# baker-laboratory/NA-MPNN

Measured on AMD Instinct MI355X. Metric: residues/sec (enc+dec fwd), N~1000 K=48 h=128; seq-recovery vs CPU ref, higher is better.
Workload: dtype f32; 1 GPU; cfg2: B=1 x N=1000 residues per rank, K=48, H=128, 3 enc + 3 dec layers, per-edge GEMMs fp32, seeded random-init weights, independent complexes per rank; precision=fp32, global_batch=1, seq_len=1000, parallelism=replicas x1

## Files before the change

na_mpnn_amd/csrc/namp_kernels.h:

```cpp
#pragma once
#include "namp_device.h"
#ifndef NAMP_MAX_LAYERS
#define NAMP_MAX_LAYERS 8
#endif

static __global__ void pack_image_kernel(const float* __restrict__ W, int ld, int col0, int OUT, int IN,
                                  float* __restrict__ img) {
  const int total = OUT * IN;
  for (int e = blockIdx.x * blockDim.x + threadIdx.x; e < total; e += gridDim.x * blockDim.x) {
    const int r = e & 3, lane = (e >> 2) & 63, t = e >> 8;
    const int ntn = OUT >> 4;
    const int tn = t % ntn, tk = t / ntn;
    const int n = 16 * tn + (lane & 15), k = 16 * tk + 4 * (lane >> 4) + r;
    img[e] = W[(size_t)n * ld + col0 + k];
  }
}

static __global__ void pack_image_bf16_kernel(const float* __restrict__ W, int ld, int col0, __bf16* __restrict__ img) {
  const int e = blockIdx.x * blockDim.x + threadIdx.x;
  if (e >= 128 * 128) return;
  const int j = e & 7, lane = (e >> 3) & 63, tn = (e >> 9) & 7, s = e >> 12;
  const int n = 16 * tn + (lane & 15), k = 32 * s + 16 * (j >> 2) + 4 * (lane >> 4) + (j & 3);
  img[e] = (__bf16)W[(size_t)n * ld + col0 + k];
}
// ... 357 lines not shown
        a0 = __builtin_elementwise_fma(w2, (f2){xv[q].x, xv[q].y}, a0);
        a1 = __builtin_elementwise_fma(w2, (f2){xv[q].z, xv[q].w}, a1);
      }
      __builtin_amdgcn_sched_barrier(0);
    }
    acc[0] = a0.x; acc[1] = a0.y; acc[2] = a1.x; acc[3] = a1.y;
    return;
  }
  f2 a2[R / 2];
#pragma unroll
  for (int q = 0; q < R / 2; ++q) a2[q] = (f2){acc[2 * q], acc[2 * q + 1]};
#pragma unroll
  for (int tk = 0; tk < 8; ++tk) {
#pragma unroll
    for (int r = 0; r < 4; ++r) {
      const float* xp = xT + (16 * tk + 4 * g + r) * R;
      const f2 w2 = (f2){wf[tk][r], wf[tk][r]};
#pragma unroll
      for (int q = 0; q < R; q += 4) {
        const f4 xv = *(const f4*)(xp + q);
        a2[q / 2] = __builtin_elementwise_fma(w2, (f2){xv.x, xv.y}, a2[q / 2]);
        a2[q / 2 + 1] = __builtin_elementwise_fma(w2, (f2){xv.z, xv.w}, a2[q / 2 + 1]);
      }
    }
    __builtin_amdgcn_sched_barrier(0);
  }
#pragma unroll
  for (int q = 0; q < R / 2; ++q) { acc[2 * q] = a2[q].x; acc[2 * q + 1] = a2[q].y; }
}

#define ROWS_TAIL_LDS_FLOATS(R) ((128 + 512 + 4 * 128 + 128) * (R) + 64 + 128 * (R))

struct ConsecutiveRows {
  int row0, nrows, G;
  __device__ __forceinline__ int operator()(int n) const { return (n < nrows && row0 + n < G) ? row0 + n : -1; }
};

template <bool SC1>
__device__ __forceinline__ void st_out(float* p, const float v) {
  if (SC1) __hip_atomic_store(p, v, __ATOMIC_RELAXED, __HIP_MEMORY_SCOPE_AGENT);
  else *p = v;
}

template <bool PF, class FragFn, class BodyFn>
__device__ __forceinline__ void tail_units(const int u0, const int total, const int step, const int lane, FragFn frag, BodyFn body,
                                           const int rot = 0) {
  if constexpr (!PF) {
#pragma unroll 1
    for (int u_ = u0; u_ < total; u_ += step) {
      const int u = (u_ + rot) & (total - 1);
      f4 wf[8];
#pragma unroll
      for (int tk = 0; tk < 8; ++tk) wf[tk] = frag(u, tk)[lane];
      body(u, wf);
    }
  } else {
    f4 wa[8], wb[8];
    int u = u0;
    if (u < total) {
#pragma unroll
      for (int tk = 0; tk < 8; ++tk) wa[tk] = frag(u, tk)[lane];
    }
#pragma unroll 1
    while (u < total) {
      int un = u + step;
      if (un < total) {
#pragma unroll
        for (int tk = 0; tk < 8; ++tk) wb[tk] = frag(un, tk)[lane];
      }
      body(u, wa);
      u = un;
      if (u >= total) break;
      un = u + step;
      if (un < total) {
#pragma unroll
        for (int tk = 0; tk < 8; ++tk) wa[tk] = frag(un, tk)[lane];
      }
      body(u, wb);
      u = un;
    }
  }
}

__device__ __forceinline__ int tail4_off(const int k, const int j) { return (((k >> 4) * 4 + ((k >> 2) & 3)) * 4 + j) * 4 + (k & 3); }

template <int NB>
__device__ __forceinline__ void tail4_x(f4 (&xr)[NB][8], const float* xB, const int lane) {
  const float* p = xB + ((lane >> 4) * 4 + (lane & 3)) * 4;
#pragma unroll
  for (int nb = 0; nb < NB; ++nb)
#pragma unroll
    for (int S = 0; S < 8; ++S) xr[nb][S] = *(const f4*)(p + nb * 512 + S * 64);
}

template <int NB>
__device__ __forceinline__ void tail4_unit(f4 (&o)[NB], const f4 (&wf)[8], const f4 (&xr)[NB][8]) {
  f4 c0[NB], c1[NB];
#ifdef NAMP_ABL_T4_NOMFMA
#pragma unroll
  for (int nb = 0; nb < NB; ++nb) {
    o[nb] = (f4){0.f, 0.f, 0.f, 0.f};
#pragma unroll
    for (int S = 0; S < 8; ++S) o[nb] += wf[S] * xr[nb][S];
  }
  return;
#endif
#pragma unroll
  for (int nb = 0; nb < NB; ++nb) { c0[nb] = (f4){0.f, 0.f, 0.f, 0.f}; c1[nb] = (f4){0.f, 0.f, 0.f, 0.f}; }
#pragma unroll
  for (int S = 0; S < 8; ++S) {
#pragma unroll
    for (int nb = 0; nb < NB; ++nb) {
      c0[nb] = __builtin_amdgcn_mfma_f32_4x4x1f32(wf[S].x, xr[nb][S].x, c0[nb], 0, 0, 0);
      c1[nb] = __builtin_amdgcn_mfma_f32_4x4x1f32(wf[S].y, xr[nb][S].y, c1[nb], 0, 0, 0);
    }
#pragma unroll
    for (int nb = 0; nb < NB; ++nb) {
      c0[nb] = __builtin_amdgcn_mfma_f32_4x4x1f32(wf[S].z, xr[nb][S].z, c0[nb], 0, 0, 0);
      c1[nb] = __builtin_amdgcn_mfma_f32_4x4x1f32(wf[S].w, xr[nb][S].w, c1[nb], 0, 0, 0);
    }
  }
#pragma unroll
  for (int nb = 0; nb < NB; ++nb) {
    f4 v = c0[nb] + c1[nb];
#pragma unroll
    for (int c = 0; c < 4; ++c) { v[c] += __shfl_xor(v[c], 16); v[c] += __shfl_xor(v[c], 32); }
    o[nb] = v;
  }
}

#define TAIL4_AHEAD 3
template <class FragFn>
__device__ __forceinline__ void tail4_request1(f4 (&wf)[8], const int u, const int lane, FragFn frag) {
#ifdef NAMP_ABL_T4_NOLOAD
#pragma unroll
  for (int tk = 0; tk < 8; ++tk) wf[tk] = (f4){1.f * u, 2.f * lane, 3.f, 4.f * tk};
  return;
#endif
#pragma unroll
  for (int tk = 0; tk < 8; ++tk) wf[tk] = frag(u, tk)[lane];
}
template <class FragFn>
__device__ __forceinline__ void tail4_request(f4 (&wf)[TAIL4_AHEAD][8], const int u0, const int total, const int step, const int lane, FragFn frag) {
#pragma unroll
  for (int t = 0; t < TAIL4_AHEAD; ++t) {
    const int u = u0 + t * step;
    tail4_request1(wf[t], u < total ? u : u0, lane, frag);
  }
}
template <class FragFn, class BodyFn, class NextFn>
__device__ __forceinline__ void tail4_phase(f4 (&wf)[TAIL4_AHEAD][8], const int u0, const int total, const int step, const int lane, FragFn frag,
                                            BodyFn body, NextFn next) {
#pragma unroll
  for (int t = 0; t < TAIL4_AHEAD; ++t) {
    const int u = u0 + t * step;
    if (u < total) body(u, wf[t]);
    next(t);
  }
  tail_units<false>(u0 + TAIL4_AHEAD * step, total, step, lane, frag, body);
}

template <int R, typename RowFn, bool SC1, bool M3, bool PF, bool AH>
__device__ __forceinline__ void node_tail_mfma4(const NodeTail& a, f4 (&x)[8], const float wsum_m, const RowFn orow, float* lds,
                                                const int tid, const int wave, const int nwaves, const int lane) {
  static_assert(R == 4 || R == 8, "node_tail_mfma4: 4 or 8 rows");
  constexpr int NB = R / 4;
  constexpr bool AHEAD = AH && !PF && R == 4;
  float* xB = lds;
  float* hB = xB + 128 * R;
  float* oP = hB + 512 * R;
  float* yT = oP + 4 * 128 * R;
  float* red = yT + 128 * R;
  float* yB = red + 64;
  const int m = lane & 15, g = lane >> 4;
  const int cb = (lane >> 2) & 3, j = lane & 3;
  const bool st_lane = lane < 16;
  const auto win_frag = [&](const int u, const int tk) { return (const f4*)a.Win_img + (tk * 32 + u) * 64; };
  const auto wout_frag = [&](const int u, const int tk) { return (const f4*)a.Wout_img + ((8 * (u >> 3) + tk) * 8 + (u & 7)) * 64; };

  NAMP_STAMP_BEGIN();
  f4 wa[AHEAD ? TAIL4_AHEAD : 1][8];
  float bin_a[TAIL4_AHEAD] = {0.f, 0.f, 0.f};
  if constexpr (AHEAD) {
    tail4_request(wa, wave, 32, nwaves, lane, win_frag);
#pragma unroll
    for (int t = 0; t < TAIL4_AHEAD; ++t) {
      const int u = wave + t * nwaves;
      bin_a[t] = a.b_in[16 * (u < 32 ? u : wave) + 4 * cb + g];
    }
  }
  if (M3 && a.m3_img) {
    if (wave == 0 && m < R) {
#pragma unroll
      for (int t = 0; t < 8; ++t) *(f4*)(xB + (m >> 2) * 512 + t * 64 + g * 16 + (m & 3) * 4) = x[t];
      if (g == 0) red[m] = wsum_m;
    }
    __syncthreads();
    {
      f4 xr[NB][8];
      tail4_x<NB>(xr, xB, lane);
      tail_units<PF>(wave, 8, nwaves, lane,
                     [&](const int u, const int tk) { return (const f4*)a.m3_img + (tk * 8 + u) * 64; },
                     [&](const int u, const f4 (&wf)[8]) {
                       f4 o[NB];
                       tail4_unit<NB>(o, wf, xr);
                       if (st_lane) {
                         const f4 b = *(const f4*)(a.m3_b + 16 * u + 4 * cb);
#pragma unroll
                         for (int nb = 0; nb < NB; ++nb) *(f4*)(oP + (4 * nb + j) * NAMP_H + 16 * u + 4 * cb) = o[nb] + b * red[4 * nb + j];
                       }
                     });
    }
    __syncthreads();
    const int mr = m < R ? m : 0;
    int hr = orow(mr);
    if (hr < 0) hr = orow(0) < 0 ? 0 : orow(0);
    const float* hsrc = a.hV + (long)hr * NAMP_H + 4 * g;
#pragma unroll
    for (int t = 0; t < 8; ++t) x[t] = *(const f4*)(hsrc + 16 * t) + *(const f4*)(oP + mr * NAMP_H + 16 * t + 4 * g);
  }

  NAMP_STAMP(7);
  layernorm_row_T(x, a.ln1_g, a.ln1_b, g);
  if (wave == 0 && m < R) {
#pragma unroll
    for (int t = 0; t < 8; ++t) *(f4*)(xB + (m >> 2) * 512 + t * 64 + g * 16 + (m & 3) * 4) = x[t];
  }
  __syncthreads();
  NAMP_STAMP(8);
  {
    f4 xr[NB][8];
    tail4_x<NB>(xr, xB, lane);
    const auto body = [&](const int u, const f4 (&wf)[8]) {
      f4 o[NB];
      tail4_unit<NB>(o, wf, xr);
      const int t_ = AHEAD ? (u - wave) / nwaves : 0;
      const float b = (AHEAD && t_ < TAIL4_AHEAD) ? (t_ == 0 ? bin_a[0] : t_ == 1 ? bin_a[1] : bin_a[2]) : a.b_in[16 * u + 4 * cb + g];
#pragma unroll
      for (int nb = 0; nb < NB; ++nb) {
        const float v = g == 0 ? o[nb].x : g == 1 ? o[nb].y : g == 2 ? o[nb].z : o[nb].w;
        hB[((u >> 3) * NB + nb) * 512 + (u & 7) * 64 + cb * 16 + j * 4 + g] = gelu_erf(v + b);
      }
    };
    if constexpr (AHEAD)
      tail4_phase(wa, wave, 32, nwaves, lane, win_frag, body, [&](const int t) {
        const int u = wave + t * nwaves;
        tail4_request1(wa[t], u < 32 ? u : wave, lane, wout_frag);
      });
    else tail_units<PF>(wave, 32, nwaves, lane, win_frag, body);
  }
  __syncthreads();
  NAMP_STAMP(9);
  {
    const auto body = [&](const int u, const f4 (&wf)[8]) {
      const int tn = u & 7, q = u >> 3;
      f4 xr[NB][8];
      tail4_x<NB>(xr, hB + q * NB * 512, lane);
      f4 o[NB];
      tail4_unit<NB>(o, wf, xr);
      if (st_lane) {
#pragma unroll
        for (int nb = 0; nb < NB; ++nb) *(f4*)(oP + (q * R + 4 * nb + j) * NAMP_H + 16 * tn + 4 * cb) = o[nb];
      }
    };
    if constexpr (AHEAD)
      tail4_phase(wa, wave, 32, nwaves, lane, wout_frag, body, [&](const int pi) {
        if (pi < a.nproj) {
          const int tn = ((wave - pi * 8) % nwaves + nwaves) % nwaves;
          const f4* img = (const f4*)(pi == 0 ? a.p[0].img : pi == 1 ? a.p[1].img : a.p[2].img) + ((tn < 8 ? tn : 0)) * 64 + lane;
#pragma unroll
          for (int tk = 0; tk < 8; ++tk) wa[pi][tk] = img[tk * 8 * 64];
        }
      });
    else tail_units<PF>(wave, 32, nwaves, lane, wout_frag, body);
  }
  __syncthreads();
  NAMP_STAMP(10);
  const int n_ = tid >> 7, c_ = tid & 127;
  const bool ln_thr = tid < 128 * R;
  const int boff = ln_thr ? (n_ >> 2) * 512 + tail4_off(c_, n_ & 3) : 0;
  float v = 0.f;
  if (ln_thr) {
    v = xB[boff] + a.b_out[c_];
#pragma unroll
    for (int q = 0; q < 4; ++q) v += oP[(q * R + n_) * NAMP_H + c_];
    float s = v;
#pragma unroll
    for (int o = 1; o < 64; o <<= 1) s += __shfl_xor(s, o);
    if (lane == 0) red[wave] = s;
  }
  __syncthreads();
  float d = 0.f;
  if (ln_thr) {
    const float mean = (red[2 * n_] + red[2 * n_ + 1]) * (1.0f / 128.0f);
    d = v - mean;
    float q = d * d;
#pragma unroll
    for (int o = 1; o < 64; o <<= 1) q += __shfl_xor(q, o);
    if (lane == 0) red[32 + wave] = q;
  }
  __syncthreads();
  if (ln_thr) {
    const float rstd = rsqrtf((red[32 + 2 * n_] + red[32 + 2 * n_ + 1]) * (1.0f / 128.0f) + 1e-5f);
    const int orw = orow(n_);
    const float mk = (a.mask && orw >= 0) ? (float)a.mask[orw] : 1.0f;
    const float y = (d * rstd * a.ln2_g[c_] + a.ln2_b[c_]) * mk;
    yT[c_ * R + n_] = y;
    yB[boff] = y;
    if (orw >= 0) st_out<SC1>(a.hV_out + (long)orw * NAMP_H + c_, y);
  }
  NAMP_STAMP(11);
  if (a.nproj == 0 && !a.head_w) return;
  __syncthreads();
  if (a.head_w) {
    for (int n = wave; n < R; n += nwaves) {
      const int orw = orow(n);
      if (orw >= 0) tail_head_row(a, yT + n, R, orw, lane);
    }
  }
  f4 xr[NB][8];
  tail4_x<NB>(xr, yB, lane);
  int orw[NB];
#pragma unroll
  for (int nb = 0; nb < NB; ++nb) orw[nb] = orow(4 * nb + j);
  auto proj_out = [&](const f4 (&o)[NB], const float* bias, const float* tok, float* out, const int tn) {
    if (!st_lane) return;
    const int c = 16 * tn + 4 * cb;
    const f4 b = bias ? *(const f4*)(bias + c) : (f4){0.f, 0.f, 0.f, 0.f};
#pragma unroll
    for (int nb = 0; nb < NB; ++nb) {
      if (orw[nb] < 0) continue;
      f4 r = o[nb] + b;
      if (tok) r += *(const f4*)(tok + (long)a.S[orw[nb]] * NAMP_H + c);
      float* dst = out + (long)orw[nb] * NAMP_H + c;
      if (SC1) { st_out<true>(dst, r.x); st_out<true>(dst + 1, r.y); st_out<true>(dst + 2, r.z); st_out<true>(dst + 3, r.w); }
      else *(f4*)dst = r;
    }
  };
  if constexpr (PF) {
    tail_units<true>(wave, 8 * (a.nproj < 2 ? a.nproj : 2), nwaves, lane,
                     [&](const int v, const int tk) { return (const f4*)((v >> 3) ? a.p[1].img : a.p[0].img) + (tk * 8 + (v & 7)) * 64; },
                     [&](const int v, const f4 (&wf)[8]) {
                       const bool second = (v >> 3) != 0;
                       f4 o[NB];
                       tail4_unit<NB>(o, wf, xr);
                       proj_out(o, second ? a.p[1].bias : a.p[0].bias, second ? a.p[1].tok : a.p[0].tok, second ? a.p[1].out : a.p[0].out, v & 7);
                     });
    NAMP_STAMP(12);
    return;
  }
#pragma unroll
  for (int pi = 0; pi < 8; ++pi) {
    if (pi >= a.nproj) break;
    const ProjDesc pd = a.p[pi];
    bool first = AHEAD && pi < TAIL4_AHEAD;
#pragma unroll 1
    for (int tn = ((wave - pi * 8) % nwaves + nwaves) % nwaves; tn < 8; tn += nwaves) {
      f4 o[NB];
      if (first) {
        tail4_unit<NB>(o, wa[pi < TAIL4_AHEAD ? pi : 0], xr);
      } else {
        f4 wf[8];
#pragma unroll
        for (int tk = 0; tk < 8; ++tk) wf[tk] = ((const f4*)pd.img)[(tk * 8 + tn) * 64 + lane];
        tail4_unit<NB>(o, wf, xr);
      }
      first = false;
      proj_out(o, pd.bias, pd.tok, pd.out, tn);
    }
  }
  NAMP_STAMP(12);
}

template <int R, typename RowFn, bool SC1 = false, bool M3 = true, bool PF = false, bool AH = false>
__device__ __forceinline__ void node_tail_rows(const NodeTail& a, f4 (&x)[8], const float wsum_m, const RowFn orow, float* lds,
                                               const int tid, const int wave, const int nwaves, const int lane) {
#ifndef NAMP_TAIL_VALU
  node_tail_mfma4<R, RowFn, SC1, M3, PF, AH>(a, x, wsum_m, orow, lds, tid, wave, nwaves, lane);
  return;
#endif
  float* xT = lds;
  float* hT = xT + 128 * R;
  float* oP = hT + 512 * R;
  float* yT = oP + 4 * 128 * R;
  float* red = yT + 128 * R;
  const int m = lane & 15, g = lane >> 4;

  NAMP_STAMP_BEGIN();
  if (M3 && a.m3_img) {
    if (wave == 0 && m < R) {
#pragma unroll
      for (int t = 0; t < 8; ++t) {
        xT[(16 * t + 4 * g + 0) * R + m] = x[t].x; xT[(16 * t + 4 * g + 1) * R + m] = x[t].y;
        xT[(16 * t + 4 * g + 2) * R + m] = x[t].z; xT[(16 * t + 4 * g + 3) * R + m] = x[t].w;
      }
      if (g == 0) red[m] = wsum_m;
    }
    __syncthreads();
#pragma unroll 1
    for (int tn = wave; tn < 8; tn += nwaves) {
      f4 wf[8];
#pragma unroll
      for (int tk = 0; tk < 8; ++tk) wf[tk] = ((const f4*)a.m3_img)[(tk * 8 + tn) * 64 + lane];
      float acc[R];
#pragma unroll
      for (int n = 0; n < R; ++n) acc[n] = 0.f;
      rows_fma<R>(acc, wf, xT, g);
#pragma unroll
      for (int n = 0; n < R; ++n) acc[n] = xg_sum(acc[n]);
      if (g == 0) {
        const float b = a.m3_b[16 * tn + m];
#pragma unroll
        for (int n = 0; n < R; ++n) yT[(16 * tn + m) * R + n] = acc[n] + b * red[n];
      }
    }
    __syncthreads();
    const int mr = m < R ? m : 0;
    int hr = orow(mr);
    if (hr < 0) hr = orow(0) < 0 ? 0 : orow(0);
    const float* hsrc = a.hV + (long)hr * NAMP_H + 4 * g;
#pragma unroll
    for (int t = 0; t < 8; ++t) {
      const float* yp = yT + (16 * t + 4 * g) * R + mr;
      x[t] = *(const f4*)(hsrc + 16 * t) + (f4){yp[0], yp[R], yp[2 * R], yp[3 * R]};
    }
  }

  NAMP_STAMP(7);
  layernorm_row_T(x, a.ln1_g, a.ln1_b, g);
  if (wave == 0 && m < R) {
#pragma unroll
    for (int t = 0; t < 8; ++t) {
      xT[(16 * t + 4 * g + 0) * R + m] = x[t].x; xT[(16 * t + 4 * g + 1) * R + m] = x[t].y;
      xT[(16 * t + 4 * g + 2) * R + m] = x[t].z; xT[(16 * t + 4 * g + 3) * R + m] = x[t].w;
    }
  }
  __syncthreads();
  NAMP_STAMP(8);
#ifdef NAMP_ABL_NOROT
  const int rot = 0;
#else
  const int rot = PF ? 0 : (int)((blockIdx.x >> 3) & 31);
#endif
#ifdef NAMP_ABL_TAILPF
  constexpr bool PFU = true;
#else
  constexpr bool PFU = PF;
#endif
  tail_units<PFU>(wave, 32, nwaves, lane,
                 [&](const int tn, const int tk) { return (const f4*)a.Win_img + (tk * 32 + tn) * 64; },
                 [&](const int tn, const f4 (&wf)[8]) {
                   float acc[R];
#pragma unroll
                   for (int n = 0; n < R; ++n) acc[n] = 0.f;
                   rows_fma<R, PF>(acc, wf, xT, g);
#pragma unroll
                   for (int n = 0; n < R; ++n) acc[n] = xg_sum(acc[n]);
                   if (g == 0) {
                     const float b = a.b_in[16 * tn + m];
#pragma unroll
                     for (int n = 0; n < R; ++n) hT[(16 * tn + m) * R + n] = gelu_erf(acc[n] + b);
// ... 248 lines not shown
    }
  }
}

enum { MODE_ENC_MSG = 0, MODE_DEC_MSG = 1, MODE_ENC_EDGE = 2, MODE_EMBED = 3 };

typedef __bf16 bf4 __attribute__((ext_vector_type(4)));
__device__ __forceinline__ int frag_off(const int t, const int g) { return 16 * t + 8 * (g & 1) + 4 * (g >> 1); }
__device__ __forceinline__ void st_frag4(__bf16* row, const int t, const int g, const f4 v) {
  *(bf4*)(row + frag_off(t, g)) = (bf4){(__bf16)v.x, (__bf16)v.y, (__bf16)v.z, (__bf16)v.w};
}

struct EdgeArgs {
  const float* hE;
  float* hE_out;
  const int32_t* E_idx;
  const int32_t* mask;
  const int32_t* mask_attend;
  const int32_t* rank;
  const float* Pa;
  const float* Pj0;
  const float* Pj1;
  const float* W1_img;
  const float* W2_img;
  const float* W3_img;
  const float* b1;
  const float* b2;
  const float* b3;
  const float* ln_g;
  const float* ln_b;
  const float* ePa; const float* ePj;
  const float* eW1_img; const float* eW2_img; const float* eW3_img;
  const float* eb2; const float* eb3;
  uint32_t drop_thresh, drop_seed; float drop_scale;
  const __bf16* hE16; __bf16* hE16_out;
  const __bf16* Pa16; const __bf16* Pj016; const __bf16* Pj116;
  float* partial;
  NodeTail tail;
  int G;
  int G_enc;
  int N, K, TPN;
};

#define EDGE_TAIL_LDS (2 * NAMP_IMG_BYTES + 12 * NAMP_H * 4 + 64 + 2048)

enum { PRE_NONE = 0, PRE_EMBED = 1, PRE_EDGE = 3 };
enum { PREC_F32 = 0, PREC_BF16 = 1, PREC_X3 = 2 };
template <int MODE, int TAIL, int PREC, int PRE, int PERSIST, class Args>
__device__ __forceinline__ void edge_stage(const Args& a, f4 (&x)[8], char* smem) {
#ifndef NAMP_ABL_NOL2PF
  f4 l2pf0 = (f4){0.f, 0.f, 0.f, 0.f}, l2pf1 = l2pf0;
#endif
  constexpr bool BF16 = (PREC == PREC_BF16);
  constexpr bool X3 = (PREC == PREC_X3);
  static_assert(PRE == PRE_NONE || (!BF16 && TAIL != 0 && (MODE == MODE_ENC_MSG || MODE == MODE_DEC_MSG)), "PRE: fp32-class message + tail only");
  constexpr bool FUSE = (PRE == PRE_EDGE);
  constexpr bool MSG = (MODE == MODE_ENC_MSG || MODE == MODE_DEC_MSG);
  constexpr bool M3_LDS = MSG && !BF16 && (TAIL == 4 || TAIL == 8);
  char* buf0 = smem;
  char* buf1 = smem + NAMP_IMG_BYTES;
  const int tid = threadIdx.x;
  const int lane = tid & 63;
  const int wave = __builtin_amdgcn_readfirstlane(tid >> 6);
  const int nwaves = blockDim.x >> 6;

  const int m = lane & 15, g = lane >> 4;
  const int npw = nwaves / a.TPN;
  const int node_l = wave / a.TPN, kt = wave - node_l * a.TPN;
  const int bid = xcd_block_index(blockIdx.x, gridDim.x);
  int node = bid * npw + node_l;
  const bool wave_active = (node_l < npw) && (node < a.G);
  if (!wave_active) node = 0;
  const int b_dec = node / a.N;
  const int i_loc = node - b_dec * a.N;
  const int node_enc = (MODE == MODE_DEC_MSG) ? ((b_dec % (a.G_enc / a.N)) * a.N + i_loc) : node;
  const int k = 16 * kt + m;
  const bool valid = wave_active && (k < a.K);
  const long erow = (long)node_enc * a.K + (valid ? k : 0);

  f4 acc[8];
  f4 ybuf[8];
  f4 (&y)[8] = PERSIST ? ybuf : x;
  f4 pjv[8];
  float w_row = 0.f;
#ifdef NAMP_ABL_NOPROLOG
#pragma unroll
  for (int t = 0; t < 8; ++t) { x[t] = (f4){0.1f * lane, 0.2f, 0.3f, 0.4f * t}; acc[t] = x[t]; pjv[t] = x[t]; }
  w_row = valid ? 1.f : 0.f;
  if (true) {
  } else if (MODE == MODE_EMBED) {
#else
  if (PERSIST != 2) {
    const float* src = a.hE + erow * NAMP_H + 4 * g;
#pragma unroll
    for (int t = 0; t < 8; ++t) x[t] = *(const f4*)(src + 16 * t);
  }
  if (MODE == MODE_EMBED) {
#endif
    if (a.ln_g) layernorm_row_T(x, a.ln_g, a.ln_b, g);
#pragma unroll
    for (int t = 0; t < 8; ++t) { acc[t] = *(const f4*)(a.b1 + 16 * t + 4 * g); pjv[t] = (f4){0.f, 0.f, 0.f, 0.f}; }
  } else if (PRE == PRE_EMBED) {
  } else if (FUSE) {
    const int j_loc = a.E_idx[erow];
    const int j = node_enc - i_loc + j_loc;
    const float* pa = a.ePa + (long)node_enc * NAMP_H + 4 * g;
    const float* pj = a.ePj + (long)j * NAMP_H + 4 * g;
#pragma unroll
    for (int t = 0; t < 8; ++t) { acc[t] = *(const f4*)(pa + 16 * t); pjv[t] = *(const f4*)(pj + 16 * t); }
  } else {
    const int j_loc = a.E_idx[erow];
    const float* pj;
    if (MODE == MODE_DEC_MSG) {
      const int j_dec = b_dec * a.N + j_loc;
      const bool bw = a.rank[j_dec] < a.rank[node];
      pj = bw ? (a.Pj0 + (long)j_dec * NAMP_H) : (a.Pj1 + (long)(node_enc - i_loc + j_loc) * NAMP_H);
      w_row = valid ? (1.0f / 30.0f) : 0.f;
    } else {
      const int j = node - i_loc + j_loc;
      pj = a.Pj0 + (long)j * NAMP_H;
      if (MODE == MODE_ENC_MSG) {
        int ma;
        if (a.mask_attend) ma = a.mask_attend[erow];
        else ma = a.mask ? (a.mask[node] * a.mask[j]) : 1;
        w_row = valid ? ((float)ma * (1.0f / 30.0f)) : 0.f;
      }
    }
    const float* pa = a.Pa + (long)node * NAMP_H + 4 * g;
    pj += 4 * g;
#pragma unroll
    for (int t = 0; t < 8; ++t) { acc[t] = *(const f4*)(pa + 16 * t); pjv[t] = *(const f4*)(pj + 16 * t); }
  }

  const f4* w0 = (const f4*)buf0 + lane;
  const f4* w1 = (const f4*)buf1 + lane;

  if (BF16) {
    const bf8* bw = (const bf8*)smem + lane;
    dma_to_lds(smem, a.W1_img, 32, wave, nwaves, lane);
    if (MODE != MODE_EMBED) dma_to_lds(smem + NAMP_BIMG_BYTES, a.W2_img, 32, wave, nwaves, lane);
    if (MODE == MODE_ENC_EDGE) dma_to_lds(smem + 2 * NAMP_BIMG_BYTES, a.W3_img, 32, wave, nwaves, lane);
    wait_dma_and_sync();
    chain_gemm_bf16<false, false>(acc, x, bw);
    if (MODE != MODE_EMBED) {
#pragma unroll
      for (int t = 0; t < 8; ++t) acc[t] += pjv[t];
      if (MSG) {
#pragma unroll
        for (int t = 0; t < 8; ++t) { const float b = a.b2[16 * t + m]; y[t] = (f4){b, b, b, b}; }
        chain_gemm_bf16<true, true>(y, acc, bw + (NAMP_BIMG_BYTES / 16));
      } else {
#pragma unroll
        for (int t = 0; t < 8; ++t) y[t] = *(const f4*)(a.b2 + 16 * t + 4 * g);
        chain_gemm_bf16<false, true>(y, acc, bw + (NAMP_BIMG_BYTES / 16));
      }
    }
  } else {
  float* cstf = (float*)(smem + 2 * NAMP_IMG_BYTES + 12 * NAMP_H * 4 + 64);
  if (FUSE) {
    dma_to_lds(buf1, a.eW1_img, 64, wave, nwaves, lane);
    dma_to_lds(buf0, a.eW2_img, 64, wave, nwaves, lane);
    for (int i = tid; i < 512; i += (int)blockDim.x) {
      const float* srcv = i < 128 ? a.eb2 : i < 256 ? a.eb3 : i < 384 ? a.ln_g : a.ln_b;
      cstf[i] = srcv[i & 127];
    }
    wait_dma_and_sync();
// ... 23 lines not shown
      for (int t = 0; t < 8; ++t) *(f4*)(dst + 16 * t) = x[t];
    }
  }
  if (PRE != PRE_NONE) {
    if (PRE == PRE_EMBED) {
      dma_to_lds(buf1, a.eW1_img, 64, wave, nwaves, lane);
      dma_to_lds(buf0, a.W1_img, 64, wave, nwaves, lane);
#pragma unroll
      for (int t = 0; t < 8; ++t) acc[t] = *(const f4*)(a.eb2 + 16 * t + 4 * g);
      wait_dma_and_sync();
      gemm128<X3, false, false>(acc, x, w1);
#pragma unroll
      for (int t = 0; t < 8; ++t) x[t] = acc[t];
      if (valid && (PERSIST == 0 || a.hE_out != nullptr)) {
        float* dst = a.hE_out + erow * NAMP_H + 4 * g;
#pragma unroll
        for (int t = 0; t < 8; ++t) *(f4*)(dst + 16 * t) = x[t];
      }
    }
#ifdef NAMP_ABL_NOTABLE2
    {
#pragma unroll
      for (int t = 0; t < 8; ++t) { acc[t] = x[t]; pjv[t] = x[t]; }
      w_row = valid ? (1.0f / 30.0f) : 0.f;
    }
    if (false)
#endif
    {
      const int j_loc = a.E_idx[erow];
      const float* pj;
      if (MODE == MODE_DEC_MSG) {
        const int j_dec = b_dec * a.N + j_loc;
        const bool bw = a.rank[j_dec] < a.rank[node];
        pj = bw ? (a.Pj0 + (long)j_dec * NAMP_H) : (a.Pj1 + (long)(node_enc - i_loc + j_loc) * NAMP_H);
        w_row = valid ? (1.0f / 30.0f) : 0.f;
      } else {
        const int j = node - i_loc + j_loc;
        pj = a.Pj0 + (long)j * NAMP_H;
        int ma;
        if (a.mask_attend) ma = a.mask_attend[erow];
        else ma = a.mask ? (a.mask[node] * a.mask[j]) : 1;
        w_row = valid ? ((float)ma * (1.0f / 30.0f)) : 0.f;
      }
      const float* pa = a.Pa + (long)node * NAMP_H + 4 * g;
      pj += 4 * g;
#pragma unroll
      for (int t = 0; t < 8; ++t) { acc[t] = *(const f4*)(pa + 16 * t); pjv[t] = *(const f4*)(pj + 16 * t); }
    }
    if (PRE == PRE_EMBED) __syncthreads();
    else wait_dma_and_sync();
    dma_to_lds(buf1, a.W2_img, 64, wave, nwaves, lane);
  } else {
  dma_to_lds(buf0, a.W1_img, 64, wave, nwaves, lane);
  if (MODE != MODE_EMBED) dma_to_lds(buf1, a.W2_img, 64, wave, nwaves, lane);
  wait_dma_and_sync();
  }
  gemm128<X3, false, false>(acc, x, w0);

  if (MODE != MODE_EMBED) {
#pragma unroll
  for (int t = 0; t < 8; ++t) acc[t] += pjv[t];
  if (MSG) {
    if (PRE != PRE_NONE) wait_dma_and_sync();
    else if (M3_LDS) __syncthreads();
    if (M3_LDS) dma_to_lds(buf0, a.W3_img, 64, wave, nwaves, lane);
#ifndef NAMP_ABL_NOL2PF
    if (TAIL == 4 || TAIL == 8) {
      const int slice = (blockIdx.x >> 3) & 31;
      const f4* p0; const f4* p1;
      if (wave < 8) {
        p0 = (const f4*)a.tail.Win_img + (slice * 8 + wave) * 64; p1 = (const f4*)a.tail.Wout_img + (slice * 8 + wave) * 64;
      } else {
        const int q = wave - 8;
        const float* img = q == 0 ? a.tail.p[0].img : q == 1 ? a.tail.p[1].img : q == 2 ? a.tail.p[2].img : a.tail.p[3].img;
        if (q >= a.tail.nproj) img = a.tail.Win_img;
        p0 = (const f4*)img + (slice * 2) * 64; p1 = p0 + 64;
      }
      l2pf0 = p0[lane]; l2pf1 = p1[lane];
    }
#endif
#pragma unroll
    for (int t = 0; t < 8; ++t) { const float b = a.b2[16 * t + m]; y[t] = (f4){b, b, b, b}; }
    gemm128<X3, true, true>(y, acc, w1);
  } else {
  if (PRE != PRE_NONE) wait_dma_and_sync();
  else __syncthreads();
  dma_to_lds(buf0, a.W3_img, 64, wave, nwaves, lane);

#pragma unroll
  for (int t = 0; t < 8; ++t) y[t] = *(const f4*)(a.b2 + 16 * t + 4 * g);
  gemm128<X3, false, true>(y, acc, w1);
  wait_dma_and_sync();
  }
  }
  }
  if (MODE == MODE_EMBED) {
    if (valid) {
      if (a.hE16_out) {
        __bf16* dst = a.hE16_out + erow * NAMP_H;
#pragma unroll
        for (int t = 0; t < 8; ++t) st_frag4(dst, t, g, acc[t]);
      } else {
        float* dst = a.hE_out + erow * NAMP_H + 4 * g;
#pragma unroll
        for (int t = 0; t < 8; ++t) *(f4*)(dst + 16 * t) = acc[t];
      }
    }
    return;
  }

  if (MODE == MODE_ENC_EDGE) {
#pragma unroll
    for (int t = 0; t < 8; ++t) acc[t] = *(const f4*)(a.b3 + 16 * t + 4 * g);
    if (BF16) chain_gemm_bf16<false, true>(acc, y, (const bf8*)smem + lane + 2 * (NAMP_BIMG_BYTES / 16));
    else      gemm128<X3, false, true>(acc, y, w0);
    if (a.drop_thresh) {
      const uint32_t key = drop_row_key(a.drop_seed, erow);
#pragma unroll
      for (int t = 0; t < 8; ++t)
#pragma unroll
        for (int r = 0; r < 4; ++r) acc[t][r] *= drop_factor(key, 16 * t + 4 * g + r, a.drop_thresh, a.drop_scale);
    }
    if (a.ln_g) {
      const float* src = a.hE + erow * NAMP_H + 4 * g;
#pragma unroll
      for (int t = 0; t < 8; ++t) acc[t] += *(const f4*)(src + 16 * t);
      layernorm_row_T(acc, a.ln_g, a.ln_b, g);
    }
    if (valid) {
      float* dst = a.hE_out + erow * NAMP_H + 4 * g;
#pragma unroll
      for (int t = 0; t < 8; ++t) *(f4*)(dst + 16 * t) = acc[t];
    }
  } else {
    float wr[4];
#pragma unroll
    for (int r = 0; r < 4; ++r) wr[r] = __shfl(w_row, 4 * g + r);
    float wsum = w_row;
#pragma unroll
    for (int o = 1; o < 16; o <<= 1) wsum += __shfl_xor(wsum, o);
    if (!TAIL) {
      float* dst = a.partial + ((long)node * a.TPN + kt) * NAMP_H + m;
#pragma unroll
      for (int t = 0; t < 8; ++t) {
        const f4 v = gelu_prec<PREC>(y[t]);
        float s = (v.x * wr[0] + v.y * wr[1]) + (v.z * wr[2] + v.w * wr[3]);
        s = xg_sum(s);
        if (wave_active && g == 0) dst[16 * t] = s;
      }
      if (wave_active && lane == 0) a.partial[(long)a.G * a.TPN * NAMP_H + (long)node * a.TPN + kt] = wsum;
    } else {
      float* dpart = (float*)(smem + 2 * NAMP_IMG_BYTES);
      float* dws = dpart + 12 * NAMP_H;
#pragma unroll
      for (int t = 0; t < 8; ++t) {
        const f4 v = gelu_prec<PREC>(y[t]);
        float s = (v.x * wr[0] + v.y * wr[1]) + (v.z * wr[2] + v.w * wr[3]);
        s = xg_sum(s);
        if (g == 0) dpart[wave * NAMP_H + 16 * t + m] = s;
      }
      if (lane == 0) dws[wave] = wsum;
#ifndef NAMP_ABL_NOL2PF
      asm volatile("" :: "v"(l2pf0), "v"(l2pf1));
#endif
      if (M3_LDS) wait_dma_and_sync();
      else __syncthreads();
      const int row0 = bid * npw;
      const int trow = row0 + m;
      const bool tvalid = (m < npw) && (trow < a.G);
      const int mm = tvalid ? m : 0;
      float wsum_m = 0.f;
#pragma unroll
      for (int t = 0; t < 8; ++t) y[t] = (f4){0.f, 0.f, 0.f, 0.f};
      for (int q = 0; q < a.TPN; ++q) {
        const float* dp = dpart + (mm * a.TPN + q) * NAMP_H + 4 * g;
#pragma unroll
        for (int t = 0; t < 8; ++t) y[t] += *(const f4*)(dp + 16 * t);
        wsum_m += dws[mm * a.TPN + q];
      }
#ifdef NAMP_ABL_NOTAIL
      if (tvalid) {
        float* dst = a.tail.hV_out + (long)trow * NAMP_H + 4 * g;
#pragma unroll
        for (int t = 0; t < 8; ++t) *(f4*)(dst + 16 * t) = y[t];
      }
      return;
#endif
#ifdef NAMP_ABL_PAIRTAIL
      if (blockIdx.x & 1) return;
#endif
      if (TAIL == 4 || TAIL == 8) {
#ifdef NAMP_ABL_PAIRTAIL
        constexpr int R = 8;
        const ConsecutiveRows orow = {row0, 2 * npw, a.G};
#else
        constexpr int R = (TAIL == 4 || TAIL == 8) ? TAIL : 4;
        const ConsecutiveRows orow = {row0, npw, a.G};
#endif
        if (M3_LDS) {
          __syncthreads();
          for (int tn = wave; tn < 8; tn += nwaves) {
            const f4 o = tile_gemm1<X3>(*(const f4*)(a.tail.m3_b + 16 * tn + 4 * g) * wsum_m, y, w0, tn);
            if (m < 8) *(f4*)(dpart + m * NAMP_H + 16 * tn + 4 * g) = o;
          }
          __syncthreads();
          const float* hsrc = a.tail.hV + (long)(row0 + mm) * NAMP_H + 4 * g;
          const float* dsrc = dpart + (mm & 7) * NAMP_H + 4 * g;
#pragma unroll
          for (int t = 0; t < 8; ++t) y[t] = *(const f4*)(hsrc + 16 * t) + *(const f4*)(dsrc + 16 * t);
          node_tail_rows<R, ConsecutiveRows, (PERSIST != 0), false, false, !BF16>(a.tail, y, 0.f, orow, (float*)smem, tid, wave, nwaves, lane);
        } else {
          node_tail_rows<R, ConsecutiveRows, (PERSIST != 0), true, false, !BF16>(a.tail, y, wsum_m, orow, (float*)smem, tid, wave, nwaves, lane);
        }
      } else {
        node_tail<false>(a.tail, y, wsum_m, row0, npw, a.G, (float*)smem, tid, wave, nwaves, lane);
      }
    }
  }
}

template <int MODE, int TAIL, int PREC = PREC_F32, int PRE = PRE_NONE>
__global__ __launch_bounds__(768) void edge_mlp_kernel(const EdgeArgs a) {
  extern __shared__ __attribute__((aligned(16))) char smem[];
  f4 x[8];
  edge_stage<MODE, TAIL, PREC, PRE, 0>(a, x, smem);
}

#define NAMP_PERSIST_MAX_STAGES 16
#define NAMP_SYNC_GROUPS 8
#define NAMP_SYNC_WORDS 64
#define NAMP_SYNC_TOP 8
#define NAMP_SYNC_GEN 16
#define NAMP_SYNC_TIMEOUT 32
#define NAMP_SYNC_DEFER 40
#ifndef NAMP_SPIN_LIMIT
#define NAMP_SPIN_LIMIT (1u << 22)
#endif

typedef __attribute__((address_space(1))) unsigned int gu32;

__device__ __forceinline__ bool spin_until_ge(gu32* word, unsigned target, gu32* tmo, unsigned code) {
  unsigned spins = 0;
  while (__hip_atomic_load(word, __ATOMIC_RELAXED, __HIP_MEMORY_SCOPE_AGENT) < target) {
    __builtin_amdgcn_s_sleep(2);
    if (++spins > NAMP_SPIN_LIMIT) {
      __hip_atomic_store(tmo, code, __ATOMIC_RELAXED, __HIP_MEMORY_SCOPE_AGENT);
      return false;
    }
  }
  return true;
}

__device__ __forceinline__ void grid_barrier(unsigned* sync, const unsigned epoch, const int tid) {
  asm volatile("s_waitcnt vmcnt(0)" ::: "memory");
  __syncthreads();
#ifdef NAMP_ABL_NOGRIDBARRIER
  return;
#endif
  if (tid == 0) {
    gu32* sy = (gu32*)sync;
    const int grp = blockIdx.x % NAMP_SYNC_GROUPS;
    const unsigned ngroups = gridDim.x < NAMP_SYNC_GROUPS ? gridDim.x : NAMP_SYNC_GROUPS;
    const unsigned in_group = (gridDim.x - grp + NAMP_SYNC_GROUPS - 1) / NAMP_SYNC_GROUPS;
#ifdef NAMP_PERSIST_RELEASE_FENCE
    __builtin_amdgcn_fence(__ATOMIC_RELEASE, "agent");
    asm volatile("s_waitcnt vmcnt(0)" ::: "memory");
#endif
    const unsigned old = __hip_atomic_fetch_add(sy + grp, 1u, __ATOMIC_RELAXED, __HIP_MEMORY_SCOPE_AGENT);
    if (old + 1 == in_group * epoch) {
      __hip_atomic_fetch_add(sy + NAMP_SYNC_TOP, 1u, __ATOMIC_RELAXED, __HIP_MEMORY_SCOPE_AGENT);
      spin_until_ge(sy + NAMP_SYNC_TOP, ngroups * epoch, sy + NAMP_SYNC_TIMEOUT, 0x10000000u | epoch);
      __hip_atomic_store(sy + NAMP_SYNC_GEN + grp, epoch, __ATOMIC_RELAXED, __HIP_MEMORY_SCOPE_AGENT);
    } else {
      spin_until_ge(sy + NAMP_SYNC_GEN + grp, epoch, sy + NAMP_SYNC_TIMEOUT, 0x20000000u | epoch);
    }
    __builtin_amdgcn_fence(__ATOMIC_ACQUIRE, "agent");
  }
  __syncthreads();
}

struct StageArgs {
  const float* hE; float* hE_out; const int32_t* E_idx; const int32_t* mask; const int32_t* rank;
  const float* Pa; const float* Pj0; const float* Pj1;
  const float* W1_img; const float* W2_img; const float* W3_img; const float* b2; const float* b3;
  const float* ln_g; const float* ln_b;
  const float* ePa; const float* ePj; const float* eW1_img; const float* eW2_img; const float* eW3_img;
  const float* eb2; const float* eb3;
  NodeTail tail;
  int G, G_enc, N, K, TPN;
  static constexpr const int32_t* mask_attend = nullptr;
  static constexpr const float* b1 = nullptr;
  static constexpr uint32_t drop_thresh = 0, drop_seed = 0;
  static constexpr float drop_scale = 1.0f;
// ... 12 lines not shown
  return (const PersistArgs*)__builtin_amdgcn_kernarg_segment_ptr();
}

template <int TAIL, int PREC>
__global__ __launch_bounds__(768) void encdec_persistent_kernel(const PersistArgs) {
  extern __shared__ __attribute__((aligned(16))) char smem[];
  const PersistArgs* P = persist_kernargs();
  const int tid = threadIdx.x;
  f4 x[8];
  if (P->embed) edge_stage<MODE_ENC_MSG, TAIL, PREC, PRE_EMBED, 1>(P->st[0], x, smem);
  else          edge_stage<MODE_ENC_MSG, TAIL, PREC, PRE_NONE, 1>(P->st[0], x, smem);
  grid_barrier(P->sync, 1, tid);
  edge_stage<MODE_ENC_MSG, TAIL, PREC, PRE_EDGE, 2>(P->st[1], x, smem);
  grid_barrier(P->sync, 2, tid);
  edge_stage<MODE_ENC_MSG, TAIL, PREC, PRE_EDGE, 2>(P->st[2], x, smem);
  grid_barrier(P->sync, 3, tid);
  edge_stage<MODE_DEC_MSG, TAIL, PREC, PRE_EDGE, 2>(P->st[3], x, smem);
  grid_barrier(P->sync, 4, tid);
  edge_stage<MODE_DEC_MSG, TAIL, PREC, PRE_NONE, 2>(P->st[4], x, smem);
  grid_barrier(P->sync, 5, tid);
  edge_stage<MODE_DEC_MSG, TAIL, PREC, PRE_NONE, 2>(P->st[5], x, smem);
  __syncthreads();
  if (__hip_atomic_load((gu32*)P->sync + NAMP_SYNC_TIMEOUT, __ATOMIC_RELAXED, __HIP_MEMORY_SCOPE_AGENT) != 0u) {
    const StageArgs& L = P->st[5];
    const int npw = (int)(blockDim.x >> 6) / L.TPN;
    const int vocab = L.tail.vocab;
    for (int e = tid; e < npw * vocab; e += blockDim.x) {
      const int node = blockIdx.x * npw + e / vocab;
      if (node < L.G && L.tail.log_probs) L.tail.log_probs[(long)node * vocab + e % vocab] = __builtin_nanf("");
    }
  }
}

struct TileMeta {
  long pa_row, pj_row; bool pj_from1;
  long erow; float w_row; int node, kt; bool valid;
};

template <int MODE>
__device__ __forceinline__ long tile_erow(const EdgeArgs& a, long tile, int m) {
  const int node = (int)((unsigned)tile / (unsigned)a.TPN);
  const int kt = (int)tile - node * a.TPN;
  const int b_dec = node / a.N;
  const int i_loc = node - b_dec * a.N;
  const int node_enc = (MODE == MODE_DEC_MSG) ? ((b_dec % (a.G_enc / a.N)) * a.N + i_loc) : node;
  const int k = 16 * kt + m;
  return (long)node_enc * a.K + (k < a.K ? k : 0);
}

template <int MODE>
__device__ __forceinline__ TileMeta tile_meta(const EdgeArgs& a, long tile, int m, int g) {
  TileMeta t;
  t.node = (int)((unsigned)tile / (unsigned)a.TPN);
  t.kt = (int)tile - t.node * a.TPN;
  const int b_dec = t.node / a.N;
  const int i_loc = t.node - b_dec * a.N;
  const int node_enc = (MODE == MODE_DEC_MSG) ? ((b_dec % (a.G_enc / a.N)) * a.N + i_loc) : t.node;
  const int k = 16 * t.kt + m;
  t.valid = k < a.K;
  t.erow = (long)node_enc * a.K + (t.valid ? k : 0);
  t.w_row = 0.f;
  const int j_loc = a.E_idx[t.erow];
  if (MODE == MODE_DEC_MSG) {
    const int j_dec = b_dec * a.N + j_loc;
    const bool bwd = a.rank[j_dec] < a.rank[t.node];
    t.pj_from1 = !bwd;
    t.pj_row = bwd ? (long)j_dec : (long)(node_enc - i_loc + j_loc);
    t.w_row = t.valid ? (1.0f / 30.0f) : 0.f;
  } else {
    const int j = t.node - i_loc + j_loc;
    t.pj_from1 = false;
    t.pj_row = j;
    if (MODE == MODE_ENC_MSG) {
      int ma;
      if (a.mask_attend) ma = a.mask_attend[t.erow];
      else ma = a.mask ? (a.mask[t.node] * a.mask[j]) : 1;
      t.w_row = t.valid ? ((float)ma * (1.0f / 30.0f)) : 0.f;
    }
  }
  t.pa_row = t.node;
  return t;
}

__device__ const int32_t g_meta_one = 1;
template <int MODE>
__device__ __forceinline__ TileMeta tile_meta_pre(const EdgeArgs& a, long tile, int m, int j_loc) {
  TileMeta t;
  t.node = (int)((unsigned)tile / (unsigned)a.TPN);
  t.kt = (int)tile - t.node * a.TPN;
  const int b_dec = t.node / a.N;
  const int i_loc = t.node - b_dec * a.N;
  const int node_enc = (MODE == MODE_DEC_MSG) ? ((b_dec % (a.G_enc / a.N)) * a.N + i_loc) : t.node;
  const int k = 16 * t.kt + m;
  t.valid = k < a.K;
  t.erow = (long)node_enc * a.K + (t.valid ? k : 0);
  t.w_row = 0.f;
  if (MODE == MODE_DEC_MSG) {
    const int j_dec = b_dec * a.N + j_loc;
    const bool bwd = a.rank[j_dec] < a.rank[t.node];
    t.pj_from1 = !bwd;
    t.pj_row = bwd ? (long)j_dec : (long)(node_enc - i_loc + j_loc);
    t.w_row = t.valid ? (1.0f / 30.0f) : 0.f;
  } else {
    const int j = t.node - i_loc + j_loc;
    t.pj_from1 = false;
    t.pj_row = j;
    if (MODE == MODE_ENC_MSG) {
      typedef const __attribute__((address_space(1))) int32_t* gptr;
      const gptr one = (gptr)&g_meta_one;
      const gptr p0 = a.mask_attend ? (gptr)(a.mask_attend + t.erow) : a.mask ? (gptr)(a.mask + t.node) : one;
      const gptr p1 = (!a.mask_attend && a.mask) ? (gptr)(a.mask + j) : one;
      const int ma = *p0 * *p1;
      t.w_row = t.valid ? ((float)ma * (1.0f / 30.0f)) : 0.f;
    }
  }
  t.pa_row = t.node;
  return t;
}

template <int MODE>
__global__ __launch_bounds__(768) void edge_mlp_bf16_persistent_kernel(const EdgeArgs a) {
  extern __shared__ __attribute__((aligned(16))) char smem[];
  const int tid = threadIdx.x, lane = tid & 63;
  const int wave = __builtin_amdgcn_readfirstlane(tid >> 6);
  const int nwaves = blockDim.x >> 6;
  const int m = lane & 15, g = lane >> 4;
  const long ntiles = (long)a.G * a.TPN;
  const long stride = (long)gridDim.x * nwaves;
  long tile = (long)blockIdx.x * nwaves + wave;
  TileMeta cur = tile_meta<MODE>(a, tile < ntiles ? tile : 0, m, g);
  f4 xn[8];
  {
    const float* src = a.hE + cur.erow * NAMP_H + 4 * g;
#pragma unroll
    for (int t = 0; t < 8; ++t) xn[t] = *(const f4*)(src + 16 * t);
  }
  float* cst = (float*)(smem + 3 * NAMP_BIMG_BYTES);
  if (MODE == MODE_ENC_EDGE && tid < 512) {
    const float* srcv = tid < 128 ? a.b2 : tid < 256 ? a.b3 : tid < 384 ? a.ln_g : a.ln_b;
    cst[tid] = srcv ? srcv[tid & 127] : 0.f;
  }
  if (MODE != MODE_ENC_EDGE && tid < 128) cst[tid] = a.b2[tid];
  const float* pa_slot = (const float*)(smem + 3 * NAMP_BIMG_BYTES + 2048 + wave * 512);
  auto pa_fetch = [&](const long row) {
    if (lane < 32)
      __builtin_amdgcn_global_load_lds((const __attribute__((address_space(1))) void*)(a.Pa + row * NAMP_H + 4 * lane),
                                       (__attribute__((address_space(3))) void*)pa_slot, 16, 0, 0);
  };
  pa_fetch(cur.pa_row);
  dma_to_lds(smem, a.W1_img, 32, wave, nwaves, lane);
  dma_to_lds(smem + NAMP_BIMG_BYTES, a.W2_img, 32, wave, nwaves, lane);
  if (MODE == MODE_ENC_EDGE) dma_to_lds(smem + 2 * NAMP_BIMG_BYTES, a.W3_img, 32, wave, nwaves, lane);
  wait_dma_and_sync();
  const bf8* bw = (const bf8*)smem + lane;
  for (; tile < ntiles; tile += stride) {
    asm volatile("" ::: "memory");
    f4 x[8], acc[8], pjv[8];
#pragma unroll
    for (int t = 0; t < 8; ++t) x[t] = xn[t];
    const TileMeta me = cur;
    asm volatile("s_waitcnt vmcnt(0)" ::: "memory");
    {
      const float* pj = (me.pj_from1 ? a.Pj1 : a.Pj0) + me.pj_row * NAMP_H + 4 * g;
#pragma unroll
      for (int t = 0; t < 8; ++t) { acc[t] = *(const f4*)(pa_slot + 16 * t + 4 * g); pjv[t] = *(const f4*)(pj + 16 * t); }
    }
    const long nt = tile + stride;
// ... 1833 lines not shown
```

Before: 2.071 million residues/s.

## Prefetch tail constants and hV rows early; pipeline projection weight loads

The node-tail parameters (layernorm gains and biases, output bias, mask, projection biases) and the hV residual rows are now loaded into registers during the edge GEMM phase. They are staged into shared memory before the tail, so the tail reads LDS instead of issuing global loads on its critical path. The projection loop also rotates its three lookahead weight buffers, requesting weights for projection pi+3 while projection pi is computed. The cost is extra register pressure (hvr, tcv) and more shared-memory use after the image region, which could lower occupancy or spill.

```diff
diff --git a/na_mpnn_amd/csrc/namp_kernels.h b/na_mpnn_amd/csrc/namp_kernels.h
--- a/na_mpnn_amd/csrc/namp_kernels.h
+++ b/na_mpnn_amd/csrc/namp_kernels.h
@@ -463,6 +463,15 @@
   }
 }
 
+__device__ const int32_t g_meta_one = 1;
+__device__ const int32_t g_meta_zero = 0;
+
+#define TC_LN1G 0
+#define TC_BOUT 256
+#define TC_LN2G 384
+#define TC_MASK 640
+#define TC_PROJ 768
+
 __device__ __forceinline__ int tail4_off(const int k, const int j) { return (((k >> 4) * 4 + ((k >> 2) & 3)) * 4 + j) * 4 + (k & 3); }
 
 template <int NB>
@@ -543,7 +552,7 @@
 
 template <int R, typename RowFn, bool SC1, bool M3, bool PF, bool AH>
 __device__ __forceinline__ void node_tail_mfma4(const NodeTail& a, f4 (&x)[8], const float wsum_m, const RowFn orow, float* lds,
-                                                const int tid, const int wave, const int nwaves, const int lane) {
+                                                const int tid, const int wave, const int nwaves, const int lane, const float* tc) {
   static_assert(R == 4 || R == 8, "node_tail_mfma4: 4 or 8 rows");
   constexpr int NB = R / 4;
   constexpr bool AHEAD = AH && !PF && R == 4;
@@ -563,13 +572,19 @@
   f4 wa[AHEAD ? TAIL4_AHEAD : 1][8];
   float bin_a[TAIL4_AHEAD] = {0.f, 0.f, 0.f};
   if constexpr (AHEAD) {
-    tail4_request(wa, wave, 32, nwaves, lane, win_frag);
 #pragma unroll
     for (int t = 0; t < TAIL4_AHEAD; ++t) {
       const int u = wave + t * nwaves;
       bin_a[t] = a.b_in[16 * (u < 32 ? u : wave) + 4 * cb + g];
     }
-  }
+    tail4_request(wa, wave, 32, nwaves, lane, win_frag);
+  }
+  const auto proj_request = [&](const int s, const ProjDesc& pd, const int pi) {
+    const int tn = ((wave - pi * 8) % nwaves + nwaves) % nwaves;
+    const f4* img = (const f4*)pd.img + (tn < 8 ? tn : 0) * 64 + lane;
+#pragma unroll
+    for (int tk = 0; tk < 8; ++tk) wa[s][tk] = img[tk * 8 * 64];
+  };
   if (M3 && a.m3_img) {
     if (wave == 0 && m < R) {
 #pragma unroll
@@ -602,7 +617,8 @@
   }
 
   NAMP_STAMP(7);
-  layernorm_row_T(x, a.ln1_g, a.ln1_b, g);
+  if constexpr (AH) layernorm_row_T(x, tc + TC_LN1G, tc + TC_LN1G + NAMP_H, g);
+  else layernorm_row_T(x, a.ln1_g, a.ln1_b, g);
   if (wave == 0 && m < R) {
 #pragma unroll
     for (int t = 0; t < 8; ++t) *(f4*)(xB + (m >> 2) * 512 + t * 64 + g * 16 + (m & 3) * 4) = x[t];
@@ -646,12 +662,7 @@
     };
     if constexpr (AHEAD)
       tail4_phase(wa, wave, 32, nwaves, lane, wout_frag, body, [&](const int pi) {
-        if (pi < a.nproj) {
-          const int tn = ((wave - pi * 8) % nwaves + nwaves) % nwaves;
-          const f4* img = (const f4*)(pi == 0 ? a.p[0].img : pi == 1 ? a.p[1].img : a.p[2].img) + ((tn < 8 ? tn : 0)) * 64 + lane;
-#pragma unroll
-          for (int tk = 0; tk < 8; ++tk) wa[pi][tk] = img[tk * 8 * 64];
-        }
+        if (pi < a.nproj) proj_request(pi, pi == 0 ? a.p[0] : pi == 1 ? a.p[1] : a.p[2], pi);
       });
     else tail_units<PF>(wave, 32, nwaves, lane, wout_frag, body);
   }
@@ -662,7 +673,7 @@
   const int boff = ln_thr ? (n_ >> 2) * 512 + tail4_off(c_, n_ & 3) : 0;
   float v = 0.f;
   if (ln_thr) {
-    v = xB[boff] + a.b_out[c_];
+    v = xB[boff] + (AH ? tc[TC_BOUT + c_] : a.b_out[c_]);
 #pragma unroll
     for (int q = 0; q < 4; ++q) v += oP[(q * R + n_) * NAMP_H + c_];
     float s = v;
@@ -684,8 +695,8 @@
   if (ln_thr) {
     const float rstd = rsqrtf((red[32 + 2 * n_] + red[32 + 2 * n_ + 1]) * (1.0f / 128.0f) + 1e-5f);
     const int orw = orow(n_);
-    const float mk = (a.mask && orw >= 0) ? (float)a.mask[orw] : 1.0f;
-    const float y = (d * rstd * a.ln2_g[c_] + a.ln2_b[c_]) * mk;
+    const float mk = AH ? tc[TC_MASK + n_] : (a.mask && orw >= 0) ? (float)a.mask[orw] : 1.0f;
+    const float y = (d * rstd * (AH ? tc[TC_LN2G + c_] : a.ln2_g[c_]) + (AH ? tc[TC_LN2G + NAMP_H + c_] : a.ln2_b[c_])) * mk;
     yT[c_ * R + n_] = y;
     yB[boff] = y;
     if (orw >= 0) st_out<SC1>(a.hV_out + (long)orw * NAMP_H + c_, y);
@@ -704,10 +715,10 @@
   int orw[NB];
 #pragma unroll
   for (int nb = 0; nb < NB; ++nb) orw[nb] = orow(4 * nb + j);
-  auto proj_out = [&](const f4 (&o)[NB], const float* bias, const float* tok, float* out, const int tn) {
+  auto proj_out = [&](const f4 (&o)[NB], const int pi, const float* bias, const float* tok, float* out, const int tn) {
     if (!st_lane) return;
     const int c = 16 * tn + 4 * cb;
-    const f4 b = bias ? *(const f4*)(bias + c) : (f4){0.f, 0.f, 0.f, 0.f};
+    const f4 b = AH ? *(const f4*)(tc + TC_PROJ + 128 * pi + c) : bias ? *(const f4*)(bias + c) : (f4){0.f, 0.f, 0.f, 0.f};
 #pragma unroll
     for (int nb = 0; nb < NB; ++nb) {
       if (orw[nb] < 0) continue;
@@ -725,7 +736,8 @@
                        const bool second = (v >> 3) != 0;
                        f4 o[NB];
                        tail4_unit<NB>(o, wf, xr);
-                       proj_out(o, second ? a.p[1].bias : a.p[0].bias, second ? a.p[1].tok : a.p[0].tok, second ? a.p[1].out : a.p[0].out, v & 7);
+                       proj_out(o, v >> 3, second ? a.p[1].bias : a.p[0].bias, second ? a.p[1].tok : a.p[0].tok, second ? a.p[1].out : a.p[0].out,
+                                v & 7);
                      });
     NAMP_STAMP(12);
     return;
@@ -734,20 +746,23 @@
   for (int pi = 0; pi < 8; ++pi) {
     if (pi >= a.nproj) break;
     const ProjDesc pd = a.p[pi];
-    bool first = AHEAD && pi < TAIL4_AHEAD;
+    int tn = ((wave - pi * 8) % nwaves + nwaves) % nwaves;
+    if constexpr (AHEAD) {
+      const int s = pi % TAIL4_AHEAD;
+      f4 o[NB];
+      if (tn < 8) tail4_unit<NB>(o, wa[s], xr);
+      if (pi + TAIL4_AHEAD < 8 && pi + TAIL4_AHEAD < a.nproj) proj_request(s, a.p[pi + TAIL4_AHEAD < 8 ? pi + TAIL4_AHEAD : 0], pi + TAIL4_AHEAD);
+      if (tn < 8) proj_out(o, pi, pd.bias, pd.tok, pd.out, tn);
+      tn += nwaves;
+    }
 #pragma unroll 1
-    for (int tn = ((wave - pi * 8) % nwaves + nwaves) % nwaves; tn < 8; tn += nwaves) {
+    for (; tn < 8; tn += nwaves) {
       f4 o[NB];
-      if (first) {
-        tail4_unit<NB>(o, wa[pi < TAIL4_AHEAD ? pi : 0], xr);
-      } else {
-        f4 wf[8];
-#pragma unroll
-        for (int tk = 0; tk < 8; ++tk) wf[tk] = ((const f4*)pd.img)[(tk * 8 + tn) * 64 + lane];
-        tail4_unit<NB>(o, wf, xr);
-      }
-      first = false;
-      proj_out(o, pd.bias, pd.tok, pd.out, tn);
+      f4 wf[8];
+#pragma unroll
+      for (int tk = 0; tk < 8; ++tk) wf[tk] = ((const f4*)pd.img)[(tk * 8 + tn) * 64 + lane];
+      tail4_unit<NB>(o, wf, xr);
+      proj_out(o, pi, pd.bias, pd.tok, pd.out, tn);
     }
   }
   NAMP_STAMP(12);
@@ -755,9 +770,9 @@
 
 template <int R, typename RowFn, bool SC1 = false, bool M3 = true, bool PF = false, bool AH = false>
 __device__ __forceinline__ void node_tail_rows(const NodeTail& a, f4 (&x)[8], const float wsum_m, const RowFn orow, float* lds,
-                                               const int tid, const int wave, const int nwaves, const int lane) {
+                                               const int tid, const int wave, const int nwaves, const int lane, const float* tc = nullptr) {
 #ifndef NAMP_TAIL_VALU
-  node_tail_mfma4<R, RowFn, SC1, M3, PF, AH>(a, x, wsum_m, orow, lds, tid, wave, nwaves, lane);
+  node_tail_mfma4<R, RowFn, SC1, M3, PF, AH>(a, x, wsum_m, orow, lds, tid, wave, nwaves, lane, tc);
   return;
 #endif
   float* xT = lds;
@@ -1172,6 +1187,9 @@
   f4 ybuf[8];
   f4 (&y)[8] = PERSIST ? ybuf : x;
   f4 pjv[8];
+  f4 hvr[8];
+  int tcv[2][2];
+  float* tc = (float*)(smem + NAMP_IMG_BYTES);
   float w_row = 0.f;
 #ifdef NAMP_ABL_NOPROLOG
 #pragma unroll
@@ -1361,6 +1379,31 @@
 #pragma unroll
     for (int t = 0; t < 8; ++t) { const float b = a.b2[16 * t + m]; y[t] = (f4){b, b, b, b}; }
     gemm128<X3, true, true>(y, acc, w1);
+    if (M3_LDS) {
+      const int hrow = bid * npw + ((m < npw && bid * npw + m < a.G) ? m : 0);
+      const float* hsrc = a.tail.hV + (long)hrow * NAMP_H + 4 * g;
+#pragma unroll
+      for (int t = 0; t < 8; ++t) hvr[t] = *(const f4*)(hsrc + 16 * t);
+      typedef const __attribute__((address_space(1))) int32_t* gi32;
+      const NodeTail& t_ = a.tail;
+#pragma unroll
+      for (int q = 0; q < 2; ++q) {
+        const int seg = wave + q * nwaves;
+#pragma unroll
+        for (int h = 0; h < 2; ++h) {
+          const int c = 64 * h + lane;
+          const float* src = seg == 0 ? t_.ln1_g : seg == 1 ? t_.ln1_b : seg == 2 ? t_.b_out : seg == 3 ? t_.ln2_g : seg == 4 ? t_.ln2_b :
+                             seg == 6 ? t_.p[0].bias : seg == 7 ? t_.p[1].bias : seg == 8 ? t_.p[2].bias : seg == 9 ? t_.p[3].bias :
+                             seg == 10 ? t_.p[4].bias : seg == 11 ? t_.p[5].bias : seg == 12 ? t_.p[6].bias : seg == 13 ? t_.p[7].bias : nullptr;
+          gi32 p = src ? (gi32)(src + c) : (gi32)&g_meta_zero;
+          if (seg == 5) {
+            const int r = bid * npw + c;
+            p = (t_.mask && c < npw && r < a.G) ? (gi32)(t_.mask + r) : (gi32)&g_meta_one;
+          }
+          tcv[q][h] = *p;
+        }
+      }
+    }
   } else {
   if (PRE != PRE_NONE) wait_dma_and_sync();
   else __syncthreads();
@@ -1476,18 +1519,25 @@
         constexpr int R = (TAIL == 4 || TAIL == 8) ? TAIL : 4;
         const ConsecutiveRows orow = {row0, npw, a.G};
 #endif
-        if (M3_LDS) {
+        if constexpr (M3_LDS) {
           __syncthreads();
+#pragma unroll
+          for (int q = 0; q < 2; ++q) {
+            const int seg = wave + q * nwaves;
+            if (seg < 6 + a.tail.nproj) {
+              tc[128 * seg + lane] = seg == 5 ? (float)tcv[q][0] : __int_as_float(tcv[q][0]);
+              tc[128 * seg + 64 + lane] = seg == 5 ? (float)tcv[q][1] : __int_as_float(tcv[q][1]);
+            }
+          }
           for (int tn = wave; tn < 8; tn += nwaves) {
             const f4 o = tile_gemm1<X3>(*(const f4*)(a.tail.m3_b + 16 * tn + 4 * g) * wsum_m, y, w0, tn);
             if (m < 8) *(f4*)(dpart + m * NAMP_H + 16 * tn + 4 * g) = o;
           }
           __syncthreads();
-          const float* hsrc = a.tail.hV + (long)(row0 + mm) * NAMP_H + 4 * g;
           const float* dsrc = dpart + (mm & 7) * NAMP_H + 4 * g;
 #pragma unroll
-          for (int t = 0; t < 8; ++t) y[t] = *(const f4*)(hsrc + 16 * t) + *(const f4*)(dsrc + 16 * t);
-          node_tail_rows<R, ConsecutiveRows, (PERSIST != 0), false, false, !BF16>(a.tail, y, 0.f, orow, (float*)smem, tid, wave, nwaves, lane);
+          for (int t = 0; t < 8; ++t) y[t] = hvr[t] + *(const f4*)(dsrc + 16 * t);
+          node_tail_rows<R, ConsecutiveRows, (PERSIST != 0), false, false, !BF16>(a.tail, y, 0.f, orow, (float*)smem, tid, wave, nwaves, lane, tc);
         } else {
           node_tail_rows<R, ConsecutiveRows, (PERSIST != 0), true, false, !BF16>(a.tail, y, wsum_m, orow, (float*)smem, tid, wave, nwaves, lane);
         }
@@ -1666,7 +1716,6 @@
   return t;
 }
 
-__device__ const int32_t g_meta_one = 1;
 template <int MODE>
 __device__ __forceinline__ TileMeta tile_meta_pre(const EdgeArgs& a, long tile, int m, int j_loc) {
   TileMeta t;
```

Result: faster. 2.101 million residues/s (median of 6 runs) (+1.5%).
